# gvanhoy/gr-liquiddsp

Hardware: AMD Instinct MI355X
Metric: Msamples/s through flex_rx (QPSK r1/2 1024B) (higher is better)
Workload: dtype f32; 1 GPU; flex_rx single stream per GPU, 20000000 samples (10 Msym), PSK4 r=1/2 (CONV_V27), 1024-B payload, CRC-24, 256-sample gaps, CFO/phase/delay + AWGN Es/N0=20 dB; frames_decoded_ok=1154, streams_per_gpu=1, blocks_in_flight=12, stage_events=none (fxrx_set_timing level 0), steps=1415, passes=independent captures (reset between passes), segments=256, repairs=0

## Files before the change

### gr-liquiddsp_amd/csrc/fx_common.h

```cpp
#pragma once
#include <stdint.h>
#include <hip/hip_vector_types.h>

#define FX_K             2
#define FX_M             7
#define FX_BETA          0.3f
#define FX_NPFB          32
#define FX_MF_TAPS       28
#define FX_PROTO_LEN     897
#define FX_PN_LEN        64
#define FX_S_LEN         156
#define FX_NFFT          512
#define FX_HOP           256
#define FX_RANGE         24
#define FX_HDR_USER      14
#define FX_HDR_DEC       20
#define FX_HDR_CRC       24
#define FX_HDR_E0        27
#define FX_HDR_ENC       54
#define FX_HDR_MOD       216
#define FX_HDR_PILOTS    15
#define FX_HDR_SYM       231
#define FX_PILOT_SPACING 16
#define FX_PROTOCOL      102
// ... 220 lines not shown
    float2   sc[1024];
    uint32_t golenc[4096];
    uint16_t h128enc[256];
    uint8_t  h74enc[16], h84enc[16], sdcol[64], sd22col[16], sd39col[32];
    uint8_t  rsexp[512], rslog[256], rsgen[40];
    float2   pn[FX_PN_LEN], pilots[16];
};

struct FxChannel {
    uint32_t th0, dl;
    float    gain, sigma;
    uint64_t seed;
};

struct FxPayJob {
    const float2 *x, *xa_end;
    int64_t  start;
    uint32_t mix_th, mix_dl; float mf_scale;
    uint32_t pfb; int32_t mfc0;
    uint32_t pll_th; float pll_f;
    uint32_t ms, bps;
    uint32_t nsym;
    uint32_t sym_off;
    uint32_t pay_len, check, fec0, fec1;
    uint32_t k;
    uint32_t l0, l1;
    uint32_t byte_off;
    uint32_t dw_off;
    uint32_t out_off;
    uint32_t pad_;
    uint32_t eq;
    uint32_t chain_idx;
    uint32_t vb_off;
    uint16_t vb_nblk;
    uint16_t vb_clean;
};
static_assert(sizeof(FxPayJob) == 128, "FxPayJob: two 64-byte lines");

#ifndef FX_VB_WARM
#define FX_VB_WARM 96
#endif

struct FxPayResult {
    uint32_t stamp[8];
};

#define FX_GANG_MAX 4
struct FxPllMember {
    const FxPayJob *jobs; const uint32_t *pll_list; const FxBlockHdr *hdr; const float2 *sym_raw; float2 *framesyms; uint8_t *hard; FxOutRec *recs;
};
struct FxPllGang { uint32_t n; FxPllMember m[FX_GANG_MAX]; };
struct FxVbpreMember {
    FxPayJob *jobs; const uint32_t *job_idx; const FxBlockHdr *hdr; const uint8_t *hard; uint8_t *bufA, *bufB, *out; FxOutRec *recs; FxBlockHdr *hdr_host;
    uint32_t first_wave, n_waves;
};
struct FxVbpreGang { uint32_t n; FxVbpreMember m[FX_GANG_MAX]; };

struct FxPlanArgs {
    const FxStreamDesc *streams; uint32_t nstreams;
    uint32_t detect, eq;
    uint32_t vb_blk;
    const FxFrame *chain; const uint32_t *chain_count;
    uint32_t *stream_base;
    FxPayJob *pjobs; FxOutRec *recs;
    uint32_t *mf_job, *mf_c0, mf_cap;
    uint32_t *pll_list, *dec_list, list_cap;
    uint32_t *vb_items, vb_cap;
    FxBlockHdr *hdr, *hdr_pay, *hdr_host;
    uint32_t *ws;
};
```

### gr-liquiddsp_amd/csrc/fx_host.cpp

```cpp
#include <hip/hip_runtime.h>
#include <algorithm>
#include <chrono>
#include <cmath>
#include <cstdio>
#include <cstdlib>
#include <cstring>
#include <memory>
#include <string>
#include <vector>
#include "../../include/fxrx.h"
#include "fx_device.h"
#include "fx_codec.hpp"
#include "fx_launch.h"
#include "fx_traffic.h"

namespace {

thread_local std::string g_err;
void set_err(const std::string &s) { g_err = s; }

#define HIP_OK(expr)                                                                          \
    do {                                                                                      \
        hipError_t e_ = (expr);                                                               \
        if (e_ != hipSuccess) {                                                               \
// ... 657 lines not shown
    std::memcpy(sl.hp_desc.p + o_streams, sds.data(), NS * sizeof(FxStreamDesc));
    const uint32_t *d_list = sl.job_list();

    const double tp2 = g_prof_on ? prof_now() : 0.0;
    if (!sl.ingest.empty()) {
        std::vector<IngestJob> todo; todo.swap(sl.ingest);
        const size_t bytes = iq_sample_bytes(sl.ingest_fmt);
        for (const IngestJob &j : todo) {
            const void *src = j.dev_src;
            if (!src) { HIP_OK(hipMemcpyAsync(sl.d_raw[j.stream].p, j.host_src, j.n * bytes, hipMemcpyHostToDevice, st)); src = sl.d_raw[j.stream].p; }
            HIP_OK(fx_launch_ingest(st, sl.ingest_fmt, src, sl.d_in[j.stream].p, (size_t)j.n, sl.ingest_scale, (unsigned)c->n_cus));
        }
    }
    HIP_OK(fx_launch_upload(st, sl.hp_desc.p, sl.d_desc.p, desc_bytes, (unsigned)c->n_cus));
    const int tl = c->timing_level >= 0 ? c->timing_level : (c->depth > 1 ? 0 : 2);
    sl.timing_level = tl;
    if (c->debug_walk_twice > 0) HIP_OK(fx_launch_prescan(st, (unsigned)spec.size(), sl.ps_words, sl.jobs(), d_list + NJ, c->d_tables));
    for (int rep = 0; rep < c->debug_walk_twice; rep++) HIP_OK(launch_walk(c, sl, st, d_list, (unsigned)early.size()));
    if (tl >= 2) HIP_OK(hipEventRecord(sl.ev[kEvStart], st));
    if (c->debug_walk_twice <= 0) HIP_OK(fx_launch_prescan(st, (unsigned)spec.size(), sl.ps_words, sl.jobs(), d_list + NJ, c->d_tables));
    HIP_OK(launch_walk(c, sl, st, d_list, (unsigned)early.size()));
    const bool verify = !detect && c->skip_seek && !sl.force_noskip;
    hipStream_t cst = st;
    if (!late.empty()) {
        if (verify) {
            HIP_OK(fx_launch_copy_u32(st, &sl.hdr_walk()->n_runs, &sl.hdr_walk()->runs_done));
            HIP_OK(launch_seekverify(c, sl, st, c->verify_per_cu * (unsigned)c->n_cus, 0u));
        }
        if (!c->st_chain) {
            int lo = 0, hi = 0;
            HIP_OK(hipDeviceGetStreamPriorityRange(&lo, &hi));
            HIP_OK(hipStreamCreateWithPriority(&c->st_chain, hipStreamNonBlocking, hi));
        }
        HIP_OK(hipEventRecord(sl.ev[kEvHandover], st));
        cst = c->st_chain;
        HIP_OK(hipStreamWaitEvent(cst, sl.ev[kEvHandover], 0));
        if (c->prev_chain) HIP_OK(hipStreamWaitEvent(cst, c->prev_chain, 0));
        HIP_OK(launch_walk(c, sl, cst, d_list + early.size(), (unsigned)late.size()));
    }
    if (tl >= 2) HIP_OK(hipEventRecord(sl.ev[kEvWalk], cst));
    if (verify)
        HIP_OK(launch_seekverify(c, sl, cst, late.empty() ? c->verify_per_cu * (unsigned)c->n_cus : (unsigned)std::min<size_t>((size_t)c->verify_per_cu * (size_t)c->n_cus, std::max<size_t>(64, 16 * late.size())), 1u));
    if (tl >= 2) HIP_OK(hipEventRecord(sl.ev[kEvVerify], cst));
    if (late.empty() && c->prev_chain) HIP_OK(hipStreamWaitEvent(cst, c->prev_chain, 0));
    if (c->carry_reader[(b + 1) % 3]) HIP_OK(hipStreamWaitEvent(cst, c->carry_reader[(b + 1) % 3], 0));
    const double tp3 = g_prof_on ? prof_now() : 0.0;
    const int rb = enqueue_back(c, sl, kChainFast, cst, may_defer);
    if (g_prof_on) { const double tp4 = prof_now(); g_prof[1] += tp1 - tp0; g_prof[2] += tp2 - tp1; g_prof[3] += tp3 - tp2; g_prof[4] += tp4 - tp3; g_prof_n++; }
    return rb;
}

static FxVbpreMember vbpre_member(Slot &sl, uint32_t first_wave, uint32_t n_waves)
{
    return FxVbpreMember{ sl.d_pjobs.p, sl.dec_list(kDecBatch), sl.hdr_pay(), sl.d_hard.p, sl.d_bufA.p, sl.d_bufB.p, sl.h_out.p, sl.h_recs.p, sl.h_hdr.p, first_wave, n_waves };
}
static int launch_tails(fxrx_ctx_s *c, Slot *const *m, unsigned n)
{
    hipStream_t st = m[n - 1]->st;
    for (unsigned i = 0; i + 1 < n; i++) HIP_OK(hipStreamWaitEvent(st, m[i]->ev[kEvMf], 0));
    auto done = [&]() -> int {
        for (unsigned i = 0; i < n; i++) { HIP_OK(hipEventRecord(m[i]->ev[kEvDone], st)); m[i]->tail_launched = true; m[i]->tail_st = st; }
        if (n > 1) { c->gang_launches++; c->gang_members += n; }
        return 0;
    };
    {
        FxPllGang g; unsigned waves[FX_GANG_MAX]; g.n = n;
        for (unsigned i = 0; i < n; i++) { const Slot &sl = *m[i]; g.m[i] = FxPllMember{ sl.d_pjobs.p, sl.d_pll_list.p, sl.hdr_pay(), sl.d_symraw.p, sl.d_symraw.p, sl.d_hard.p, sl.h_recs.p }; waves[i] = sl.tail.pll_waves; }
        HIP_OK(fx_launch_paypll(&g, waves, c->pll_waves, st, c->d_tables));
    }
    for (unsigned i = 0; i < n; i++) if (m[i]->timing_level >= 1) HIP_OK(hipEventRecord(m[i]->ev[kEvPll], st));
    if (c->debug_stop_after == 6) return done();
    for (unsigned i = 0; i < n; i++) {
        Slot &sl = *m[i];
        if (c->cfg.soft_decision) {
            HIP_OK(fx_launch_softdemod(sl.tail.mf_grid, st, sl.d_pjobs.p, sl.d_mf_job.p, sl.d_mf_c0.p, sl.hdr_pay(), sl.d_symraw.p, sl.d_hard.p, sl.d_soft.p, c->d_tables));
            if (c->cfg.want_framesyms) HIP_OK(hipMemcpyAsync(sl.h_soft.p, sl.d_soft.p, 8 * sl.byte_cap, hipMemcpyDeviceToHost, st));
        }
        HIP_OK(launch_decoders(c, sl, st, 0u, sl.tail.plain, sl.tail.rs));
    }
    {
        FxVbpreGang g; g.n = n;
        for (unsigned i = 0; i < n; i++) g.m[i] = vbpre_member(*m[i], 0u, m[i]->vb_blk ? m[i]->tail.vb_pre : 0u);
        HIP_OK(fx_launch_vbpre(&g, st, c->d_tables, c->vb_clean ? 1 : 0, c->vb_early_tail && c->vb_clean ? 1 : 0));
    }
    for (unsigned i = 0; i < n; i++) {
        Slot &sl = *m[i];
        if (sl.vb_blk) HIP_OK(launch_trellis(c, sl, st, sl.tail.vb_items, sl.tail.vb_packed, sl.tail.with_fix, sl.tail.vb_fin, sl.tail.fb));
        if (sl.timing_level >= 2) HIP_OK(hipEventRecord(sl.ev[kEvDec], st));
        if (c->cfg.want_framesyms) HIP_OK(fx_launch_symcopy(2u * (unsigned)c->n_cus, st, sl.hdr_pay(), sl.d_symraw.p, sl.h_framesyms.p));
    }
    return done();
}

static int close_gang(fxrx_ctx_s *c)
{
    if (c->gang.empty()) return 0;
    if (c->gang.size() > FX_GANG_MAX) { set_err("open gang larger than FX_GANG_MAX (internal error)"); return FXRX_ERR_STATE; }
    Slot *m[FX_GANG_MAX]; unsigned n = 0;
    for (Slot *s : c->gang) m[n++] = s;
    c->gang.clear();
    return launch_tails(c, m, n);
}

static int enqueue_back(fxrx_ctx_s *c, Slot &sl, int chain_mode, hipStream_t chain_st, bool may_defer)
{
    const unsigned NS = c->cfg.n_streams; const bool detect = c->cfg.mode == FXRX_MODE_DETECTOR;
    const uint64_t b = sl.seq; const uint32_t chain_slots = sl.chain_cap; hipStream_t st = sl.st;
// ... 631 lines not shown
```

### gr-liquiddsp_amd/csrc/fx_kernels.hip

```cpp
#include <hip/hip_runtime.h>
#include <algorithm>
#include "fx_device.h"
#include "fx_launch.h"
#include "fx_vbclean.h"
#include "fx_rsgmd.h"

#define HALF         256

template <int WW> struct WalkLdsT {
    static constexpr int WAVES = WW;
    static constexpr bool SWEEP_PAIRS = WW == 4;
    float2 win[FX_NFFT];
    float2 X[FX_NFFT];
    float2 S[FX_NFFT];
    float2 scr[WW][576];
    float2 v[640];
    float2 P[256];
    float  m2[FX_NFFT];
    float2 hdr[FX_HDR_SYM];
    float2 cw[(WW + 1) * FX_HOP + 8];
    __device__ __forceinline__ float2 *scr2(int wave) { return wave < 2 ? v + 576 * wave : cw + 576 * (wave - 2); }
    float2 pb[16];
    float2 eqw[16];
    float  taps[FX_MF_TAPS];
// ... 1967 lines not shown
        __threadfence();
        __hip_atomic_store(&pw[PW_FLAG + wg], 2u, __ATOMIC_RELEASE, __HIP_MEMORY_SCOPE_AGENT);
    }
    __syncthreads();
    uint32_t before[PLAN_NV];
#pragma unroll
    for (int q = 0; q < PLAN_NV; q++) before[q] = base_s[q];
    for (uint32_t c0 = g0; c0 < g1; c0 += PLAN_THREADS) {
        const uint32_t g = c0 + tid;
        const bool live = g < g1;
        uint32_t v[PLAN_NV], tot[PLAN_NV]; PlanWords w;
        PlanFrame f = plan_frame(g, live, a, w, v);
        plan_scan<PLAN_THREADS>(v, tot, ws);
#pragma unroll
        for (int q = 0; q < PLAN_NV; q++) { v[q] += before[q]; before[q] += tot[q]; }
        if (f.batch && plan_demote(v[PV_VB], f.vnb, a.vb_cap)) { f.batch = false; f.vnb = 0; }
        if (live) {
            plan_emit(a.pjobs + g, a.recs + g, plan_rest(f.fp, a.streams + f.sidx), w, f, v, a.eq, (uint32_t)(f.fp - a.chain), 0u);
            for (uint32_t c = 0; c < f.nblk; c++) if (v[PV_MF] + c < a.mf_cap) { a.mf_job[v[PV_MF] + c] = g; a.mf_c0[v[PV_MF] + c] = c * 1024u; }
        }
        {
            const PlanKey key = plan_key(w.ms, w.fec0, w.fec1);
            (void)wave_agg_add(pw + PW_CLS_CNT, key.cls, 1u, f.valid);
            (void)wave_agg_add(pw + PW_DEC_CNT, key.dec(f.batch), 1u, f.valid);
            (void)wave_agg_add(pw + PW_VBC_CNT, key.vc, f.vnb, f.batch);
        }
        __syncthreads();
    }
}

extern "C" __global__ __launch_bounds__(PLAN_THREADS)
void fx_planlists_kernel(const FxPlanArgs a)
{
    __shared__ struct { FxBlockHdr h; uint32_t cls_base[FX_PLL_CLASSES + 1], vbc_base[8], last; } sh;
    uint32_t *const pw = a.ws;
    const PlanCounts<true> cnt{ pw + PW_CLS_CNT, pw + PW_DEC_CNT, pw + PW_VBC_CNT };
    const int tid = threadIdx.x;
    const uint32_t N = __hip_atomic_load(&a.stream_base[a.nstreams], __ATOMIC_RELAXED, __HIP_MEMORY_SCOPE_AGENT);
    if (tid == 0) plan_class_bases(cnt, sh.cls_base, sh.vbc_base);
    __syncthreads();
    uint32_t g0, g1; plan_range(N, g0, g1);
    for (uint32_t c0 = g0; c0 < g1; c0 += PLAN_THREADS) {
        const uint32_t g = c0 + tid;
        const bool live = g < g1;
        uint32_t ms = 0, fec0 = 0, fec1 = 0, vnb = 0; bool val = false;
        if (live) { const FxPayJob &j = a.pjobs[g]; val = j.pad_ != 0; ms = j.ms; fec0 = j.fec0; fec1 = j.fec1; vnb = j.vb_nblk; }
        const PlanKey key = plan_key(ms, fec0, fec1);
        const bool bt = val && vnb;
        const uint32_t pp = sh.cls_base[key.cls] + wave_agg_add(pw + PW_CLS_FILL, key.cls, 1u, val);
        if (val && pp < a.list_cap) a.pll_list[pp] = g;
        const uint32_t rs = key.dec(bt), dp = wave_agg_add(pw + PW_DEC_FILL, rs, 1u, val);
        if (val && dp < a.list_cap) a.dec_list[(size_t)rs * a.list_cap + dp] = g;
        const uint32_t at = sh.vbc_base[key.vc] + wave_agg_add(pw + PW_VBC_FILL, key.vc, vnb, bt);
        if (bt) {
            for (uint32_t b = 0; b < vnb; b++) if (at + b < a.vb_cap) { a.vb_items[at + b] = g; a.vb_items[a.vb_cap + at + b] = b; }
            a.pjobs[g].vb_off = at;
        }
    }
    if (blockIdx.x == 0) plan_pad_lists<PLAN_THREADS>(cnt, sh.cls_base, sh.vbc_base, a);
    __threadfence(); __syncthreads();
    if (tid == 0) sh.last = atomicAdd(&pw[PW_TICKET], 1u) == gridDim.x - 1 ? 1u : 0u;
    __syncthreads();
    if (!sh.last) return;
    __threadfence();
    if (tid == 0) {
        sh.h = *a.hdr;
        plan_fill_hdr(sh.h, N, (const volatile uint32_t *)(pw + PW_INC + 8 * (gridDim.x - 1)), cnt, sh.cls_base, sh.vbc_base, a);
    }
    __syncthreads();
    plan_mirror_hdr<PLAN_THREADS>(sh.h, a);
    for (int i = tid; i < PW_WORDS; i += PLAN_THREADS) pw[i] = 0u;
}

#define PLAN_TILE 2048
#define PLAN_BATCH 2
#define PLAN_LDS_STREAMS 256
enum { PO_CLS = 0, PO_DEC = FX_PLL_CLASSES, PO_VBC = FX_PLL_CLASSES + 4, PO_N = FX_PLL_CLASSES + 12 };
template <int NT> struct PlanOneShared {
    FxBlockHdr h;
    uint32_t ws[NT / 64][PLAN_NV];
    uint32_t cnt[PO_N], fill[PO_N];
    uint32_t cls_base[FX_PLL_CLASSES + 1], vbc_base[8];
    uint32_t sbase[PLAN_LDS_STREAMS + 1], cbase[PLAN_LDS_STREAMS];
};
template <int NT> __device__ __forceinline__ uint32_t plan_one_slot(uint32_t g, const FxPlanArgs &a, const PlanOneShared<NT> &sh, uint32_t &sidx)
{
    if (a.nstreams <= PLAN_LDS_STREAMS) { sidx = plan_stream_of(sh.sbase, a.nstreams, g); return sh.cbase[sidx] + (g - sh.sbase[sidx]); }
    sidx = plan_stream_of(a.stream_base, a.nstreams, g);
    return a.streams[sidx].chain_base + (g - a.stream_base[sidx]);
}

template <int NT> __global__ __launch_bounds__(NT)
void fx_planfused_kernel(const FxPlanArgs a)
{
    constexpr uint32_t TILE = PLAN_TILE;
    constexpr int KEEP = PLAN_TILE / NT, JB = PLAN_BATCH;
    static_assert(NT % 64 == 0 && KEEP * NT == PLAN_TILE && KEEP % JB == 0, "whole waves; the tile is KEEP frames a thread, in whole batches");
    __shared__ PlanOneShared<NT> sh;
    __shared__ uint4 keep[PLAN_TILE];
    const PlanCounts<false> cnt{ sh.cnt + PO_CLS, sh.cnt + PO_DEC, sh.cnt + PO_VBC };
    const uint32_t tid = threadIdx.x, nstreams = a.nstreams;
#ifdef FX_STAMPS
    unsigned long long tk_ = __builtin_readcyclecounter(); uint32_t st1_ = 0, st2_ = 0, st6_ = 0, st7_ = 0;
#define PLAN_TICK(acc) do { const unsigned long long t_ = __builtin_readcyclecounter(); acc += (uint32_t)(t_ - tk_); tk_ = t_; } while (0)
#else
#define PLAN_TICK(acc) do { } while (0)
#endif
    {
        const uint32_t *src = reinterpret_cast<const uint32_t *>(a.hdr); uint32_t *dst = reinterpret_cast<uint32_t *>(&sh.h);
        for (int i = (int)tid; i < (int)(sizeof(FxBlockHdr) / 4); i += NT) dst[i] = src[i];
        if (tid < PO_N) { sh.cnt[tid] = 0u; sh.fill[tid] = 0u; }
        if (tid <= FX_PLL_CLASSES) sh.cls_base[tid] = 0u;
        if (tid < 8) sh.vbc_base[tid] = 0u;
    }
    uint32_t N;
    if (nstreams <= PLAN_LDS_STREAMS) {
        uint32_t v[PLAN_NV] = { tid < nstreams ? a.chain_count[tid] : 0u, 0, 0, 0, 0, 0, 0 }, tot[PLAN_NV];
        if (nstreams > 1) plan_scan<NT>(v, tot, sh.ws); else { tot[0] = v[0]; v[0] = 0u; }
        if (tid < nstreams) { sh.sbase[tid] = v[0]; a.stream_base[tid] = v[0]; sh.cbase[tid] = a.streams[tid].chain_base; }
        if (tid == 0) { sh.sbase[nstreams] = tot[0]; a.stream_base[nstreams] = tot[0]; }
        __syncthreads();
        N = sh.sbase[nstreams];
    } else N = plan_stream_bases<NT>(a.chain_count, nstreams, a.stream_base, sh.ws);

    uint32_t run[PLAN_NV] = { 0, 0, 0, 0, 0, 0, 0 };
    for (int pass = N > TILE ? 0 : 1; pass < 2; pass++) {
#pragma unroll
        for (int q = 0; q < PLAN_NV; q++) run[q] = 0u;
        for (uint32_t t0 = 0; t0 < N; t0 += TILE) {
            const uint32_t nt = min(TILE, N - t0), t1 = t0 + nt, per = (nt + NT - 1) / NT, f0 = t0 + tid * per;
            uint32_t st[PLAN_NV];
            PlanWords w[KEEP]; uint32_t slot[KEEP], sidx[KEEP];
#pragma unroll
            for (int i = 0; i < KEEP; i++) {
                const bool live = (uint32_t)i < per && f0 + i < t1;
                slot[i] = plan_one_slot(live ? f0 + i : t0, a, sh, sidx[i]);
                w[i] = plan_words(a.chain + slot[i]);
            }
#pragma unroll
            for (int q = 0; q < PLAN_NV; q++) st[q] = 0u;
#pragma unroll
            for (int i = 0; i < KEEP; i++) {
                uint32_t v[PLAN_NV];
                (void)plan_sizes(w[i], (uint32_t)i < per && f0 + i < t1, a.detect, a.vb_blk, v);
#pragma unroll
                for (int q = 0; q < PLAN_NV; q++) st[q] += v[q];
            }
            {
                uint32_t tot[PLAN_NV];
                plan_scan<NT>(st, tot, sh.ws);
#pragma unroll
                for (int q = 0; q < PLAN_NV; q++) { st[q] += run[q]; run[q] += tot[q]; }
            }
            if (pass == 0 || N <= TILE) {
                uint32_t vb = st[PV_VB];
#pragma unroll
                for (int i = 0; i < KEEP; i++) {
                    uint32_t v[PLAN_NV];
                    const PlanFrame f = plan_sizes(w[i], (uint32_t)i < per && f0 + i < t1, a.detect, a.vb_blk, v);
                    const bool batch = f.batch && !plan_demote(vb, f.vnb, a.vb_cap);
                    vb += f.vnb;
                    if (f.valid) {
                        const PlanKey key = plan_key(w[i].ms, w[i].fec0, w[i].fec1);
                        atomicAdd(&sh.cnt[PO_CLS + key.cls], 1u);
                        atomicAdd(&sh.cnt[PO_DEC + key.dec(batch)], 1u);
                        if (batch) atomicAdd(&sh.cnt[PO_VBC + key.vc], f.vnb);
                    }
                }
            }
            if (pass == 0) continue;
            if (t0 == 0) {
                __syncthreads();
                if (tid == 0) plan_class_bases(cnt, sh.cls_base, sh.vbc_base);
                __syncthreads();
            }
            PLAN_TICK(st1_);
#pragma unroll
            for (int b0 = 0; b0 < KEEP; b0 += JB) {
                if ((uint32_t)b0 >= per) break;
                PlanRest r[JB];
#pragma unroll
                for (int i = 0; i < JB; i++) r[i] = plan_rest(a.chain + slot[b0 + i], a.streams + sidx[b0 + i]);
#pragma unroll
                for (int i = 0; i < JB; i++) {
                    const uint32_t g = f0 + b0 + i;
                    if ((uint32_t)(b0 + i) >= per || g >= t1) break;
                    const PlanWords &wi = w[b0 + i];
                    uint32_t v[PLAN_NV];
                    PlanFrame f = plan_sizes(wi, true, a.detect, a.vb_blk, v);
                    f.fp = a.chain + slot[b0 + i]; f.sidx = sidx[b0 + i];
                    if (f.batch && plan_demote(st[PV_VB], f.vnb, a.vb_cap)) { f.batch = false; f.vnb = 0; }
                    uint32_t at = 0;
                    if (f.valid) {
                        const PlanKey key = plan_key(wi.ms, wi.fec0, wi.fec1);
                        const uint32_t pp = sh.cls_base[key.cls] + atomicAdd(&sh.fill[PO_CLS + key.cls], 1u);
                        if (pp < a.list_cap) a.pll_list[pp] = g;
                        const uint32_t rs = key.dec(f.batch), dp = atomicAdd(&sh.fill[PO_DEC + rs], 1u);
                        if (dp < a.list_cap) a.dec_list[(size_t)rs * a.list_cap + dp] = g;
                        if (f.batch) at = sh.vbc_base[key.vc] + atomicAdd(&sh.fill[PO_VBC + key.vc], f.vnb);
                    }
                    keep[g - t0] = make_uint4(at, f.vnb, st[PV_MF], f.nblk);
                    plan_emit(a.pjobs + g, a.recs + g, r[i], wi, f, st, a.eq, slot[b0 + i], at);
#pragma unroll
                    for (int q = 0; q < PLAN_NV; q++) st[q] += v[q];
                }
            }
            __syncthreads();
            PLAN_TICK(st2_);
            for (uint32_t k = tid >> 4; k < nt; k += NT / 16) {
                const uint4 kp = keep[k];
                const uint32_t g = t0 + k, sub = tid & 15u;
                for (uint32_t b = sub; b < kp.y; b += 16u) if (kp.x + b < a.vb_cap) { a.vb_items[kp.x + b] = g; a.vb_items[a.vb_cap + kp.x + b] = b; }
                for (uint32_t c = sub; c < kp.w; c += 16u) if (kp.z + c < a.mf_cap) { a.mf_job[kp.z + c] = g; a.mf_c0[kp.z + c] = c * 1024u; }
            }
            __syncthreads();
        }
    }
    plan_pad_lists<NT>(cnt, sh.cls_base, sh.vbc_base, a);
    PLAN_TICK(st6_);
    __threadfence(); __syncthreads();
    PLAN_TICK(st7_);
    if (tid == 0) {
#ifdef FX_STAMPS
        sh.h.stamp[1] = st1_; sh.h.stamp[2] = st2_; sh.h.stamp[6] = st6_; sh.h.stamp[7] = st7_;
#endif
        plan_fill_hdr(sh.h, N, run, cnt, sh.cls_base, sh.vbc_base, a);
    }
    __syncthreads();
    plan_mirror_hdr<NT>(sh.h, a);
}

extern "C" hipError_t fx_launch_plan(hipStream_t st, unsigned grid, int fused, unsigned threads, const FxPlanArgs &a)
{
    const unsigned g = grid < 1u ? 1u : (grid > PLAN_MAXG ? PLAN_MAXG : grid);
    if (fused && g == 1u) {
        if (threads == 512u) hipLaunchKernelGGL((fx_planfused_kernel<512>), dim3(1), dim3(512), 0, st, a);
        else if (threads == 256u) hipLaunchKernelGGL((fx_planfused_kernel<256>), dim3(1), dim3(256), 0, st, a);
        else return hipErrorInvalidValue;
    } else {
        hipLaunchKernelGGL(fx_plan_kernel, dim3(g), dim3(PLAN_THREADS), 0, st, a);
        hipLaunchKernelGGL(fx_planlists_kernel, dim3(g), dim3(PLAN_THREADS), 0, st, a);
    }
    return hipGetLastError();
}
extern "C" unsigned fx_plan_ws_words(void) { return PW_WORDS; }

#define PMF_THREADS 256
#define PMF_SYMS    1024
#define PMF_SPAN    (2 * PMF_SYMS + FX_MF_TAPS)

__global__ __launch_bounds__(PMF_THREADS)
void fx_paymf_kernel(const FxPayJob *jobs, const uint32_t *blk_job, const uint32_t *blk_c0, const FxBlockHdr *hdr, const FxFrame *chain, float2 *sym_raw,
                     const FxTables *T)
{
    constexpr int LEAD = FX_EQ_TAPS - 1;
    __shared__ float2 v[PMF_SPAN + LEAD + 4];
    __shared__ float2 u[2 * PMF_SYMS + FX_EQ_TAPS];
    __shared__ float2 eqw[16];
    __shared__ float taps[FX_MF_TAPS];
    const uint32_t nitems = hdr->n_mfblk;
    const int tid = threadIdx.x;
    const float2 *sc = T->sc;
    for (uint32_t bi = blockIdx.x; bi < nitems; bi += gridDim.x) {
        const FxPayJob job = jobs[blk_job[bi]];
        const uint32_t c0 = blk_c0[bi];
        const uint32_t ns = min((uint32_t)PMF_SYMS, job.nsym - c0);
// ... 1575 lines not shown
    row[8] = q2.x; row[9] = q2.y; row[10] = q2.z; row[11] = q2.w; row[12] = q3.x; row[13] = q3.y; row[14] = q3.z; row[15] = q3.w;
    lbase = o << 3;
}
__device__ __forceinline__ void vb2_forward(int p, uint32_t blk, const VbHalf &A, const VbHalf &B, uint32_t *lds)
{
    uint32_t Q[64], N[64];
#pragma unroll
    for (int i = 0; i < 64; i++) Q[i] = 0u;
    unsigned pa, pb; conv_punct(p, pa, pb);
    const unsigned up = (unsigned)p;
    const uint32_t warm = vb_warm(p);
    VbStream sa = vb_stream_at(A.first ? A.t_reg : A.t_reg - warm, up), sb = vb_stream_at(B.first ? B.t_reg : B.t_reg - warm, up);
    const auto lo = [&](int i) { return (Q[i] & 0xFFFFu) >> 1; };
    const auto hi = [&](int i) { return Q[i] >> 17; };
    uint32_t *rowa = lds + (threadIdx.x & 63) * VB_ROW, *rowb = lds + (64 + (threadIdx.x & 63)) * VB_ROW;
    uint32_t la = 0, lb = 0;
    const uint32_t nsteps = warm + blk;
    for (uint32_t u = 0; u < nsteps; u += 2) {
        if (u == warm) {
            if (A.first) {
#pragma unroll
                for (int i = 0; i < 64; i++) Q[i] = (Q[i] & 0xFFFF0000u) | (i ? 1024u : 0u);
            } else if (A.on) vb_save_vec(lo, A.vec);
            if (B.first) {
#pragma unroll
                for (int i = 0; i < 64; i++) Q[i] = (Q[i] & 0x0000FFFFu) | (i ? 1024u << 16 : 0u);
            } else if (B.on) vb_save_vec(hi, B.vec);
        }
        if ((u & 127u) == 0u) { vb_stage(A.enc, sa.nb, A.on, rowa, la); vb_stage(B.enc, sb.nb, B.on, rowb, lb); }
        if ((u & 15u) == 0u) {
            const uint32_t ia = (sa.nb - la) >> 5, ib = (sb.nb - lb) >> 5;
            sa.w0 = __builtin_bswap32(rowa[ia]); sa.w1 = __builtin_bswap32(rowa[ia + 1]); sa.wbase = la + (ia << 5);
            sb.w0 = __builtin_bswap32(rowb[ib]); sb.w1 = __builtin_bswap32(rowb[ib + 1]); sb.wbase = lb + (ib << 5);
        }
        const bool in_reg = u >= warm;
        const bool run_a = in_reg || !A.first, run_b = in_reg || !B.first;
        unsigned long long a0, b0, a1, b1;
        vb2_step(Q, N, pa, pb, up, sa, sb, run_a, run_b, a0, b0);
        vb2_step(N, Q, pa, pb, up, sa, sb, run_a, run_b, a1, b1);
        const uint32_t ur = u - warm;
        if (in_reg && ur < (uint32_t)FX_VB_TWARM) {
            if (A.on && A.t_reg + ur < A.t1) { A.dwl[(size_t)ur * 64u] = a0; A.dwl[(size_t)(ur + 1u) * 64u] = a1; }
            if (B.on && B.t_reg + ur < B.t1) { B.dwl[(size_t)ur * 64u] = b0; B.dwl[(size_t)(ur + 1u) * 64u] = b1; }
        } else {
            if (A.on && in_reg && A.t_reg + ur < A.t1) { __builtin_nontemporal_store(a0, A.dwl + (size_t)ur * 64u); __builtin_nontemporal_store(a1, A.dwl + (size_t)(ur + 1u) * 64u); }
            if (B.on && in_reg && B.t_reg + ur < B.t1) { __builtin_nontemporal_store(b0, B.dwl + (size_t)ur * 64u); __builtin_nontemporal_store(b1, B.dwl + (size_t)(ur + 1u) * 64u); }
        }
    }
    if (A.on) vb_save_vec(lo, A.vec + 64);
    if (B.on) vb_save_vec(hi, B.vec + 64);
}

struct VbItem { uint32_t g, b, t_reg, t1, Tn, nblk; bool on; };
__device__ __forceinline__ VbItem vb_item(const FxPayJob *jobs, const uint32_t *vb_items, uint32_t item_cap, uint32_t slot, uint32_t blk)
{
    VbItem it;
    const uint32_t item = vb_items[slot];
    it.on = item != 0xFFFFFFFFu;
    it.g = it.on ? item : 0u; it.b = it.on ? vb_items[item_cap + slot] : 0u;
    const FxPayJob &job = jobs[it.g];
    it.on = it.on && job.vb_clean == 0u;
    it.Tn = 8u * job.k + 6u; it.nblk = job.vb_nblk;
    it.t_reg = it.b * blk; it.t1 = min(it.Tn, it.t_reg + blk);
    return it;
}
struct VbWaveItem { VbItem it; uint32_t slot; unsigned long long *dwl; uint8_t *vec; };
__device__ __forceinline__ VbWaveItem vb_wave_item(const FxPayJob *jobs, const uint32_t *vb_items, uint32_t item_cap, uint32_t slot, uint32_t blk,
                                                   unsigned long long *dwv, uint8_t *vec_arena)
{
    VbWaveItem w;
    w.slot = slot; w.it = vb_item(jobs, vb_items, item_cap, slot, blk);
    w.dwl = vb_slab(dwv, slot, blk); w.vec = vec_arena ? vec_arena + (size_t)slot * 128u : nullptr;
    return w;
}
__device__ __forceinline__ int vb_wave_period(unsigned long long live, unsigned fec0)
{
    return conv_p((unsigned)__shfl((int)fec0, __ffsll((long long)live) - 1, 64));
}

extern "C" __global__ __launch_bounds__(64, 3)
void fx_vbfwd_kernel(const FxPayJob *jobs, const uint32_t *vb_items, uint32_t item_cap, const FxBlockHdr *hdr, uint32_t first_item, const uint8_t *bufB,
                     unsigned long long *dwv, uint8_t *vec_arena, uint32_t *vb_st)
{
    const uint32_t nitems = hdr->n_vb_items, blk = hdr->vb_blk;
    const uint32_t it0 = first_item + blockIdx.x * 128u;
    if (it0 >= nitems) return;
    const uint32_t slot_a = it0 + threadIdx.x, slot_b = slot_a + 64u;
    const VbItem ia = vb_item(jobs, vb_items, item_cap, slot_a, blk);
    VbItem ib = ia; ib.on = false;
    if (slot_b < nitems) ib = vb_item(jobs, vb_items, item_cap, slot_b, blk);
    const unsigned long long live_a = __ballot(ia.on), live_b = __ballot(ib.on);
    if (!live_a && !live_b) return;
    const FxPayJob &ja = jobs[ia.g], &jb = jobs[ib.g];
    const int p = live_a ? vb_wave_period(live_a, ja.fec0) : vb_wave_period(live_b, jb.fec0);
    VbHalf A, B;
    A.enc = bufB + ja.byte_off; A.on = ia.on; A.first = !ia.on || ia.b == 0; A.t_reg = A.first && !ia.on ? 0u : ia.t_reg; A.t1 = ia.t1;
    A.dwl = vb_slab(dwv, slot_a, blk); A.vec = vec_arena + (size_t)slot_a * 128u;
    B.enc = bufB + jb.byte_off; B.on = ib.on; B.first = !ib.on || ib.b == 0; B.t_reg = B.first && !ib.on ? 0u : ib.t_reg; B.t1 = ib.t1;
    B.dwl = vb_slab(dwv, ib.on ? slot_b : slot_a, blk); B.vec = vec_arena + (size_t)(ib.on ? slot_b : slot_a) * 128u;
    __shared__ uint32_t rows[128 * VB_ROW];
    vb2_forward(p, blk, A, B, rows);
    if (ia.on) vb_st[slot_a] = vb_st_fresh(vb_make_guess(A.dwl, ia.t1 - ia.t_reg), false);
    if (ib.on) vb_st[slot_b] = vb_st_fresh(vb_make_guess(B.dwl, ib.t1 - ib.t_reg), false);
}

extern "C" __global__ __launch_bounds__(64)
void fx_vbfwd1_kernel(const FxPayJob *jobs, const uint32_t *vb_items, uint32_t item_cap, const FxBlockHdr *hdr, uint32_t first_item, const uint8_t *bufB,
                      unsigned long long *dwv, uint8_t *vec_arena, uint32_t *vb_st)
{
    const uint32_t nitems = hdr->n_vb_items, blk = hdr->vb_blk;
    const uint32_t it0 = first_item + blockIdx.x * 64u;
    if (it0 >= nitems) return;
    const VbWaveItem w = vb_wave_item(jobs, vb_items, item_cap, it0 + threadIdx.x, blk, dwv, vec_arena);
    const VbItem &it = w.it;
    const unsigned long long live = __ballot(it.on);
    if (!live) return;
    const FxPayJob &job = jobs[it.g];
    const int p = vb_wave_period(live, job.fec0);
    const bool first = !it.on || it.b == 0;
    vb_forward(bufB + job.byte_off, p, it.t_reg, it.t1, first ? 1 : 0, nullptr, w.dwl, first ? nullptr : w.vec, w.vec + 64,
               vb_warm(p) + blk, vb_warm(p), it.on);
    if (it.on) vb_st[w.slot] = vb_st_fresh(vb_make_guess(w.dwl, it.t1 - it.t_reg), false);
}

__device__ __forceinline__ bool vb_same64(const uint8_t *a, const uint8_t *b)
{
    const uint4 *pa = reinterpret_cast<const uint4 *>(a), *pb = reinterpret_cast<const uint4 *>(b);
    bool same = true;
#pragma unroll
    for (int i = 0; i < 4; i++) { const uint4 x = pa[i], y = pb[i]; same = same && x.x == y.x && x.y == y.y && x.z == y.z && x.w == y.w; }
    return same;
}

extern "C" __global__ __launch_bounds__(64)
void fx_vbfix_kernel(const FxPayJob *jobs, const uint32_t *vb_items, uint32_t item_cap, const FxBlockHdr *hdr, uint32_t first_item, const uint8_t *bufB,
                     unsigned long long *dwv, uint8_t *vec_arena, uint32_t *vb_st, uint32_t dbg)
{
    const uint32_t nitems = hdr->n_vb_items, blk = hdr->vb_blk;
    const uint32_t it0 = first_item + blockIdx.x * 64u;
    if (it0 >= nitems) return;
    const VbWaveItem w = vb_wave_item(jobs, vb_items, item_cap, it0 + threadIdx.x, blk, dwv, vec_arena);
    const VbItem &it = w.it;
    uint8_t *vec = w.vec;
    const bool bad = it.on && it.b > 0 && !vb_same64(vec, vec - 64) && !((dbg & 2u) && (w.slot & 1u));
    const unsigned long long fails = __ballot(bad);
    if (!fails) return;
    const FxPayJob &job = jobs[it.g];
    const int p = vb_wave_period(fails, job.fec0);
    vb_forward(bufB + job.byte_off, p, it.t_reg, it.t1, 2, bad ? vec - 64 : vec, w.dwl, vec, vec + 64, blk, 0u, bad);
    if (bad) vb_st[w.slot] = vb_st_fresh(vb_make_guess(w.dwl, it.t1 - it.t_reg), true);
}

__device__ __forceinline__ void vb_trace16(const unsigned long long *dwl, uint32_t u0, uint32_t lim, unsigned &st, uint32_t &bits16)
{
    unsigned long long q[16];
#pragma unroll
    for (int i = 0; i < 16; i++) q[i] = (u0 + (uint32_t)i < lim) ? dwl[(size_t)(u0 + (uint32_t)i) * 64u] : 0ull;
#pragma unroll
    for (int i = 15; i >= 0; i--) {
        if (u0 + (uint32_t)i < lim) {
            bits16 |= (st & 1u) << i;
            st = (st >> 1) | ((unsigned)((q[i] >> st) & 1ull) << 5);
        }
    }
}
__device__ __forceinline__ unsigned vb_trace_chunk(const unsigned long long *dwl, uint32_t c, uint32_t len, unsigned st, uint32_t &b0, uint32_t &b1)
{
    unsigned long long bits = 0;
#pragma unroll 1
    for (int grp = 3; grp >= 0; grp--) {
        uint32_t b16 = 0;
        vb_trace16(dwl, 64u * c + 16u * (uint32_t)grp, len, st, b16);
        bits |= (unsigned long long)b16 << (16 * grp);
    }
    b0 = (uint32_t)bits; b1 = (uint32_t)(bits >> 32);
    return st;
}

extern "C" __global__ __launch_bounds__(64)
void fx_vbtrace_kernel(const FxPayJob *jobs, const uint32_t *vb_items, uint32_t item_cap, const FxBlockHdr *hdr, uint32_t first_item, uint8_t *bufA,
                       unsigned long long *dwv, uint32_t *vb_st, uint32_t dbg)
{
    const uint32_t nitems = hdr->n_vb_items, blk = hdr->vb_blk;
    const uint32_t it0 = first_item + blockIdx.x * 64u;
    if (it0 >= nitems) return;
    const VbWaveItem w = vb_wave_item(jobs, vb_items, item_cap, it0 + threadIdx.x, blk, dwv, nullptr);
    const VbItem &it = w.it;
    const uint32_t slot = w.slot;
    if (!__ballot(it.on)) return;
    const FxPayJob &job = jobs[it.g];
    const uint32_t len = it.on ? it.t1 - it.t_reg : 0u;
    const uint32_t old = it.on ? vb_st[slot] : 0u;
    const unsigned long long *dwl = w.dwl;
    const bool has_next = it.on && it.b + 1u < it.nblk;
    const unsigned S = (has_next && !(dbg & 1u)) ? vb_st_guess(vb_st[slot + 1u]) : 0u;
    uint8_t *A = bufA + job.byte_off + it.t_reg / 8u;
    unsigned st = S;
    for (int c = (int)(blk / 64u) - 1; c >= 0; c--) {
        if (!__any(64u * (uint32_t)c < len)) continue;
        uint32_t b0, b1;
        st = vb_trace_chunk(dwl, (uint32_t)c, len, st, b0, b1);
        if (64u * (uint32_t)c < len) vb_emit(A, (uint32_t)c, b0, b1);
    }
    if (it.on) vb_st[slot] = vb_st_traced(old, S, st);
}

struct VbSlabTracer {
    static constexpr uint32_t max_chunks = 64u;
    const unsigned long long *dwl; uint32_t len;
    template <int NCH>
    __device__ __forceinline__ void operator()(const uint32_t (&cidx)[NCH], const bool (&act)[NCH], unsigned (&st)[NCH], uint32_t (&bits)[NCH][2]) const
    {
#pragma unroll
        for (int j = 0; j < NCH; j++) if (act[j]) st[j] = vb_trace_chunk(dwl, cidx[j], len, st[j], bits[j][0], bits[j][1]);
    }
};
__device__ __forceinline__ unsigned vb_retrace_block(const unsigned long long *dwl, uint32_t len, unsigned end_state, uint8_t *dec, uint8_t *scratch, int lane)
{
    const VbSlabTracer trace = { dwl, len };
    const unsigned arrived = vb_traceback<1>(trace, (len + 63) / 64, end_state, dec, scratch, lane);
    __threadfence_block(); __builtin_amdgcn_wave_barrier();
    return arrived;
}

template <bool IN_LDS>
__device__ __forceinline__ void vbpre_front(const FxPayJob &job, const uint8_t *hs, uint8_t *X, uint8_t *A, uint8_t *B, const FxTables *T, int lane)
{
    uint8_t *W = IN_LDS ? X : A;
    pack_bytes_wave(hs, job.bps, job.l1, W, lane);
    if (!IN_LDS) __threadfence_block();
    __builtin_amdgcn_wave_barrier();
    deinterleave_wave(W, job.l1, lane);
    if (!IN_LDS || job.fec1 != FX_FEC_NONE) {
        if (IN_LDS) {
            for (uint32_t j = lane; j < job.l1; j += DEC_THREADS) A[j] = X[j];
            __threadfence_block(); __builtin_amdgcn_wave_barrier();
        }
        block_fec_decode<false>(job.fec1, job.l0, A, B, T, lane);
        __threadfence_block(); __builtin_amdgcn_wave_barrier();
        if (IN_LDS) {
            for (uint32_t j = lane; j < job.l0; j += DEC_THREADS) X[j] = B[j];
            __builtin_amdgcn_wave_barrier();
        } else W = B;
    }
    deinterleave_wave(W, job.l0, lane);
    if (lane < (IN_LDS ? 16 : 8)) W[job.l0 + lane] = 0;
}
__device__ __forceinline__ uint64_t vb_lds_word(const uint8_t *X, uint32_t w)
{
    const uint2 v = reinterpret_cast<const uint2 *>(X)[w];
    return ((uint64_t)__builtin_bswap32(v.x) << 32) | __builtin_bswap32(v.y);
}
__device__ __forceinline__ bool vb_clean_check(FxPayJob *jobs, uint32_t jf, uint32_t k, const uint8_t *X, uint8_t *A, int lane)
{
    const uint32_t Tn = 8u * k + 6u, nw = (Tn + 31u) / 32u;
    bool ok = true;
    for (uint32_t w = lane; w < nw; w += DEC_THREADS) {
        uint32_t u;
        ok = ok && vbc_check_word(w >= 2u ? vb_lds_word(X, w - 2u) : 0ull, w >= 1u ? vb_lds_word(X, w - 1u) : 0ull, vb_lds_word(X, w), w, Tn, u) == 0u;
    }
    const bool clean = !__any(!ok);
    if (clean) {
        for (uint32_t w = lane; 4u * w < k; w += DEC_THREADS) {
            uint32_t u;
            (void)vbc_check_word(w >= 2u ? vb_lds_word(X, w - 2u) : 0ull, w >= 1u ? vb_lds_word(X, w - 1u) : 0ull, vb_lds_word(X, w), w, Tn, u);
            reinterpret_cast<uint32_t *>(A)[w] = __builtin_bswap32(u);
        }
    }
    if (lane == 0) jobs[jf].vb_clean = clean ? 1u : 0u;
    return clean;
}
extern "C" __global__ __launch_bounds__(DEC_THREADS)
void fx_vbpre_kernel(const FxVbpreGang g, const FxTables *T, uint32_t clean_on, uint32_t early_tail)
{
    __shared__ __attribute__((aligned(16))) uint8_t X[DEC_LDS];
    const FxVbpreMember m = g.m[blockIdx.y];
    if (blockIdx.x >= m.n_waves) return;
    const uint32_t njobs = m.hdr->n_dec_batch;
    const uint32_t ji = m.first_wave + blockIdx.x;
    if (ji >= njobs) return;
    FxPayJob *jobs = m.jobs; const uint8_t *hard = m.hard; uint8_t *bufA = m.bufA, *bufB = m.bufB, *out = m.out;
    FxOutRec *recs = m.recs; FxBlockHdr *hdr_host = m.hdr_host;
    const int lane = threadIdx.x & 63;
    const uint32_t jf = m.job_idx[ji];
    FxPayJob job = jobs[jf];
    job.l0 = __builtin_amdgcn_readfirstlane(job.l0); job.l1 = __builtin_amdgcn_readfirstlane(job.l1);
    job.fec1 = __builtin_amdgcn_readfirstlane(job.fec1); job.bps = __builtin_amdgcn_readfirstlane(job.bps);
    uint8_t *A = bufA + job.byte_off, *B = bufB + job.byte_off;
    const uint8_t *hs = hard + job.sym_off;
    if (vbpre_lds_fits(job.l1, job.l0)) {
        vbpre_front<true>(job, hs, X, A, B, T, lane);
        __builtin_amdgcn_wave_barrier();
        const uint32_t n16 = (job.l0 + 8u + 15u) / 16u;
        for (uint32_t j = lane; j < n16; j += DEC_THREADS) reinterpret_cast<uint4 *>(B)[j] = reinterpret_cast<const uint4 *>(X)[j];
        job.k = __builtin_amdgcn_readfirstlane(job.k);
        const bool clean = clean_on && conv_p(job.fec0) == 1 && vb_clean_check(jobs, jf, job.k, X, A, lane);
        if (!early_tail) return;
        if (!clean) { if (lane == 0) hdr_host->vb_dirty = 1u; return; }
        job.pay_len = __builtin_amdgcn_readfirstlane(job.pay_len); job.check = __builtin_amdgcn_readfirstlane(job.check);
        __threadfence_block(); __builtin_amdgcn_wave_barrier();
        dec_tail(job, jf, A, lane, out, recs, FX_REC_VB_CLEAN);
        return;
    }
    vbpre_front<false>(job, hs, nullptr, A, B, T, lane);
    if (early_tail && lane == 0) hdr_host->vb_dirty = 1u;
}

extern "C" __global__ __launch_bounds__(64)
void fx_vbfinish_kernel(const FxPayJob *jobs, const uint32_t *job_idx, FxBlockHdr *hdr, uint32_t first_wave, uint8_t *bufA, uint8_t *bufB,
                        unsigned long long *dwv, const uint8_t *vec_arena, const uint32_t *vb_st, uint32_t *fb_list, uint32_t list_cap, uint8_t *out, FxOutRec *recs,
                        FxBlockHdr *hdr_host, uint32_t early_tail)
{
    const uint32_t njobs = hdr->n_dec_batch, blk = hdr->vb_blk;
    const uint32_t ji = first_wave + blockIdx.x;
    if (ji >= njobs) return;
    const int lane = threadIdx.x & 63;
    const uint32_t jf = job_idx[ji];
    FxPayJob job = jobs[jf];
    job.k = __builtin_amdgcn_readfirstlane(job.k); job.pay_len = __builtin_amdgcn_readfirstlane(job.pay_len);
    job.check = __builtin_amdgcn_readfirstlane(job.check); job.vb_nblk = (uint16_t)__builtin_amdgcn_readfirstlane(job.vb_nblk);
    job.vb_off = __builtin_amdgcn_readfirstlane(job.vb_off); job.vb_clean = (uint16_t)__builtin_amdgcn_readfirstlane(job.vb_clean);
    uint8_t *A = bufA + job.byte_off, *B = bufB + job.byte_off;
    if (job.vb_clean) { if (!early_tail) dec_tail(job, jf, A, lane, out, recs, FX_REC_VB_CLEAN); return; }
    const uint32_t at = job.vb_off, nblk = job.vb_nblk;
    bool bad = false, mism = false; uint32_t rep = 0;
    for (uint32_t base = 0; base < nblk; base += 64) {
        const uint32_t b = base + (uint32_t)lane;
        const uint32_t v = b < nblk ? vb_st[at + b] : 0u, vn = b + 1u < nblk ? vb_st[at + b + 1u] : 0u;
        if (b > 0 && b < nblk) { const uint8_t *vec = vec_arena + (size_t)(at + b) * 128u; const bool same = vb_same64(vec, vec - 64); bad = bad || !same; }
        rep += (uint32_t)__popcll(__ballot(vb_st_repeated(v)));
        mism = mism || (b + 1u < nblk && vb_st_end(v) != vb_st_arrived(vn));
    }
    if (__any(bad)) {
        if (lane == 0) { const uint32_t s = atomicAdd(&hdr->n_vb_fallback, 1u); if (s < list_cap) fb_list[s] = jf; hdr_host->vb_ticket = 1u; }
        return;
    }
    if (__any(mism)) {
        unsigned need = vb_st_arrived(vb_st[at + nblk - 1u]);
        for (int b = (int)nblk - 2; b >= 0; b--) {
            const uint32_t v = vb_st[at + (uint32_t)b];
            if (vb_st_end(v) != need) need = vb_retrace_block(vb_slab(dwv, at + (uint32_t)b, blk), blk, need, A + (size_t)b * (blk / 8u), B, lane);
            else need = vb_st_arrived(v);
        }
    }
    __threadfence_block(); __builtin_amdgcn_wave_barrier();
    dec_tail(job, jf, A, lane, out, recs, rep << 8);
}

extern "C" hipError_t fx_launch_vbpre(const FxVbpreGang *gang, hipStream_t st, const FxTables *T, int clean_on, int early_tail)
{
    if (gang->n > FX_GANG_MAX) return hipErrorInvalidValue;
    FxVbpreGang g; g.n = 0;
    unsigned gw = 0;
    for (uint32_t i = 0; i < gang->n; i++) if (gang->m[i].n_waves) { g.m[g.n++] = gang->m[i]; gw = gang->m[i].n_waves > gw ? gang->m[i].n_waves : gw; }
    if (g.n == 0) return hipSuccess;
    for (uint32_t i = g.n; i < FX_GANG_MAX; i++) g.m[i] = g.m[0];
    hipLaunchKernelGGL(fx_vbpre_kernel, dim3(gw, g.n), dim3(DEC_THREADS), 0, st, g, T, clean_on ? 1u : 0u, early_tail ? 1u : 0u);
// ... 405 lines not shown
```

Measured before the change: 40680 Msamples/s.

## Write Viterbi block item lists in vbpre, skipping entries for clean frames

```diff
diff --git a/gr-liquiddsp_amd/csrc/fx_common.h b/gr-liquiddsp_amd/csrc/fx_common.h
--- a/gr-liquiddsp_amd/csrc/fx_common.h
+++ b/gr-liquiddsp_amd/csrc/fx_common.h
@@ -296,6 +296,7 @@
 struct FxPllGang { uint32_t n; FxPllMember m[FX_GANG_MAX]; };
 struct FxVbpreMember {
     FxPayJob *jobs; const uint32_t *job_idx; const FxBlockHdr *hdr; const uint8_t *hard; uint8_t *bufA, *bufB, *out; FxOutRec *recs; FxBlockHdr *hdr_host;
+    uint32_t *vb_items; uint32_t vb_cap;
     uint32_t first_wave, n_waves;
 };
 struct FxVbpreGang { uint32_t n; FxVbpreMember m[FX_GANG_MAX]; };
diff --git a/gr-liquiddsp_amd/csrc/fx_host.cpp b/gr-liquiddsp_amd/csrc/fx_host.cpp
--- a/gr-liquiddsp_amd/csrc/fx_host.cpp
+++ b/gr-liquiddsp_amd/csrc/fx_host.cpp
@@ -733,7 +733,7 @@
 
 static FxVbpreMember vbpre_member(Slot &sl, uint32_t first_wave, uint32_t n_waves)
 {
-    return FxVbpreMember{ sl.d_pjobs.p, sl.dec_list(kDecBatch), sl.hdr_pay(), sl.d_hard.p, sl.d_bufA.p, sl.d_bufB.p, sl.h_out.p, sl.h_recs.p, sl.h_hdr.p, first_wave, n_waves };
+    return FxVbpreMember{ sl.d_pjobs.p, sl.dec_list(kDecBatch), sl.hdr_pay(), sl.d_hard.p, sl.d_bufA.p, sl.d_bufB.p, sl.h_out.p, sl.h_recs.p, sl.h_hdr.p, sl.d_vb_items.p, sl.vb_cap, first_wave, n_waves };
 }
 static int launch_tails(fxrx_ctx_s *c, Slot *const *m, unsigned n)
 {
diff --git a/gr-liquiddsp_amd/csrc/fx_kernels.hip b/gr-liquiddsp_amd/csrc/fx_kernels.hip
--- a/gr-liquiddsp_amd/csrc/fx_kernels.hip
+++ b/gr-liquiddsp_amd/csrc/fx_kernels.hip
@@ -2043,10 +2043,7 @@
         const uint32_t rs = key.dec(bt), dp = wave_agg_add(pw + PW_DEC_FILL, rs, 1u, val);
         if (val && dp < a.list_cap) a.dec_list[(size_t)rs * a.list_cap + dp] = g;
         const uint32_t at = sh.vbc_base[key.vc] + wave_agg_add(pw + PW_VBC_FILL, key.vc, vnb, bt);
-        if (bt) {
-            for (uint32_t b = 0; b < vnb; b++) if (at + b < a.vb_cap) { a.vb_items[at + b] = g; a.vb_items[a.vb_cap + at + b] = b; }
-            a.pjobs[g].vb_off = at;
-        }
+        if (bt) a.pjobs[g].vb_off = at;
     }
     if (blockIdx.x == 0) plan_pad_lists<PLAN_THREADS>(cnt, sh.cls_base, sh.vbc_base, a);
     __threadfence(); __syncthreads();
@@ -2088,7 +2085,7 @@
     constexpr int KEEP = PLAN_TILE / NT, JB = PLAN_BATCH;
     static_assert(NT % 64 == 0 && KEEP * NT == PLAN_TILE && KEEP % JB == 0, "whole waves; the tile is KEEP frames a thread, in whole batches");
     __shared__ PlanOneShared<NT> sh;
-    __shared__ uint4 keep[PLAN_TILE];
+    __shared__ uint2 keep[PLAN_TILE];
     const PlanCounts<false> cnt{ sh.cnt + PO_CLS, sh.cnt + PO_DEC, sh.cnt + PO_VBC };
     const uint32_t tid = threadIdx.x, nstreams = a.nstreams;
 #ifdef FX_STAMPS
@@ -2190,7 +2187,7 @@
                         if (dp < a.list_cap) a.dec_list[(size_t)rs * a.list_cap + dp] = g;
                         if (f.batch) at = sh.vbc_base[key.vc] + atomicAdd(&sh.fill[PO_VBC + key.vc], f.vnb);
                     }
-                    keep[g - t0] = make_uint4(at, f.vnb, st[PV_MF], f.nblk);
+                    keep[g - t0] = make_uint2(st[PV_MF], f.nblk);
                     plan_emit(a.pjobs + g, a.recs + g, r[i], wi, f, st, a.eq, slot[b0 + i], at);
 #pragma unroll
                     for (int q = 0; q < PLAN_NV; q++) st[q] += v[q];
@@ -2199,10 +2196,9 @@
             __syncthreads();
             PLAN_TICK(st2_);
             for (uint32_t k = tid >> 4; k < nt; k += NT / 16) {
-                const uint4 kp = keep[k];
+                const uint2 kp = keep[k];
                 const uint32_t g = t0 + k, sub = tid & 15u;
-                for (uint32_t b = sub; b < kp.y; b += 16u) if (kp.x + b < a.vb_cap) { a.vb_items[kp.x + b] = g; a.vb_items[a.vb_cap + kp.x + b] = b; }
-                for (uint32_t c = sub; c < kp.w; c += 16u) if (kp.z + c < a.mf_cap) { a.mf_job[kp.z + c] = g; a.mf_c0[kp.z + c] = c * 1024u; }
+                for (uint32_t c = sub; c < kp.y; c += 16u) if (kp.x + c < a.mf_cap) { a.mf_job[kp.x + c] = g; a.mf_c0[kp.x + c] = c * 1024u; }
             }
             __syncthreads();
         }
@@ -3884,24 +3880,26 @@
 }
 
 struct VbItem { uint32_t g, b, t_reg, t1, Tn, nblk; bool on; };
-__device__ __forceinline__ VbItem vb_item(const FxPayJob *jobs, const uint32_t *vb_items, uint32_t item_cap, uint32_t slot, uint32_t blk)
+__device__ __forceinline__ VbItem vb_item(const FxPayJob *jobs, const uint32_t *vb_items, uint32_t item_cap, uint32_t slot, uint32_t blk, uint32_t nframes)
 {
     VbItem it;
     const uint32_t item = vb_items[slot];
-    it.on = item != 0xFFFFFFFFu;
-    it.g = it.on ? item : 0u; it.b = it.on ? vb_items[item_cap + slot] : 0u;
+    it.on = item < nframes;
+    it.g = it.on ? item : 0u;
     const FxPayJob &job = jobs[it.g];
-    it.on = it.on && job.vb_clean == 0u;
+    const uint32_t b = slot - job.vb_off;
+    it.on = it.on && job.vb_clean == 0u && b < job.vb_nblk && vb_items[item_cap + slot] == b;
+    it.b = it.on ? b : 0u;
     it.Tn = 8u * job.k + 6u; it.nblk = job.vb_nblk;
     it.t_reg = it.b * blk; it.t1 = min(it.Tn, it.t_reg + blk);
     return it;
 }
 struct VbWaveItem { VbItem it; uint32_t slot; unsigned long long *dwl; uint8_t *vec; };
-__device__ __forceinline__ VbWaveItem vb_wave_item(const FxPayJob *jobs, const uint32_t *vb_items, uint32_t item_cap, uint32_t slot, uint32_t blk,
+__device__ __forceinline__ VbWaveItem vb_wave_item(const FxPayJob *jobs, const uint32_t *vb_items, uint32_t item_cap, uint32_t slot, uint32_t blk, uint32_t nframes,
                                                    unsigned long long *dwv, uint8_t *vec_arena)
 {
     VbWaveItem w;
-    w.slot = slot; w.it = vb_item(jobs, vb_items, item_cap, slot, blk);
+    w.slot = slot; w.it = vb_item(jobs, vb_items, item_cap, slot, blk, nframes);
     w.dwl = vb_slab(dwv, slot, blk); w.vec = vec_arena ? vec_arena + (size_t)slot * 128u : nullptr;
     return w;
 }
@@ -3914,13 +3912,13 @@
 void fx_vbfwd_kernel(const FxPayJob *jobs, const uint32_t *vb_items, uint32_t item_cap, const FxBlockHdr *hdr, uint32_t first_item, const uint8_t *bufB,
                      unsigned long long *dwv, uint8_t *vec_arena, uint32_t *vb_st)
 {
-    const uint32_t nitems = hdr->n_vb_items, blk = hdr->vb_blk;
+    const uint32_t nitems = hdr->n_vb_items, blk = hdr->vb_blk, nframes = hdr->n_frames;
     const uint32_t it0 = first_item + blockIdx.x * 128u;
     if (it0 >= nitems) return;
     const uint32_t slot_a = it0 + threadIdx.x, slot_b = slot_a + 64u;
-    const VbItem ia = vb_item(jobs, vb_items, item_cap, slot_a, blk);
+    const VbItem ia = vb_item(jobs, vb_items, item_cap, slot_a, blk, nframes);
     VbItem ib = ia; ib.on = false;
-    if (slot_b < nitems) ib = vb_item(jobs, vb_items, item_cap, slot_b, blk);
+    if (slot_b < nitems) ib = vb_item(jobs, vb_items, item_cap, slot_b, blk, nframes);
     const unsigned long long live_a = __ballot(ia.on), live_b = __ballot(ib.on);
     if (!live_a && !live_b) return;
     const FxPayJob &ja = jobs[ia.g], &jb = jobs[ib.g];
@@ -3940,10 +3938,10 @@
 void fx_vbfwd1_kernel(const FxPayJob *jobs, const uint32_t *vb_items, uint32_t item_cap, const FxBlockHdr *hdr, uint32_t first_item, const uint8_t *bufB,
                       unsigned long long *dwv, uint8_t *vec_arena, uint32_t *vb_st)
 {
-    const uint32_t nitems = hdr->n_vb_items, blk = hdr->vb_blk;
+    const uint32_t nitems = hdr->n_vb_items, blk = hdr->vb_blk, nframes = hdr->n_frames;
     const uint32_t it0 = first_item + blockIdx.x * 64u;
     if (it0 >= nitems) return;
-    const VbWaveItem w = vb_wave_item(jobs, vb_items, item_cap, it0 + threadIdx.x, blk, dwv, vec_arena);
+    const VbWaveItem w = vb_wave_item(jobs, vb_items, item_cap, it0 + threadIdx.x, blk, nframes, dwv, vec_arena);
     const VbItem &it = w.it;
     const unsigned long long live = __ballot(it.on);
     if (!live) return;
@@ -3968,10 +3966,10 @@
 void fx_vbfix_kernel(const FxPayJob *jobs, const uint32_t *vb_items, uint32_t item_cap, const FxBlockHdr *hdr, uint32_t first_item, const uint8_t *bufB,
                      unsigned long long *dwv, uint8_t *vec_arena, uint32_t *vb_st, uint32_t dbg)
 {
-    const uint32_t nitems = hdr->n_vb_items, blk = hdr->vb_blk;
+    const uint32_t nitems = hdr->n_vb_items, blk = hdr->vb_blk, nframes = hdr->n_frames;
     const uint32_t it0 = first_item + blockIdx.x * 64u;
     if (it0 >= nitems) return;
-    const VbWaveItem w = vb_wave_item(jobs, vb_items, item_cap, it0 + threadIdx.x, blk, dwv, vec_arena);
+    const VbWaveItem w = vb_wave_item(jobs, vb_items, item_cap, it0 + threadIdx.x, blk, nframes, dwv, vec_arena);
     const VbItem &it = w.it;
     uint8_t *vec = w.vec;
     const bool bad = it.on && it.b > 0 && !vb_same64(vec, vec - 64) && !((dbg & 2u) && (w.slot & 1u));
@@ -4013,10 +4011,10 @@
 void fx_vbtrace_kernel(const FxPayJob *jobs, const uint32_t *vb_items, uint32_t item_cap, const FxBlockHdr *hdr, uint32_t first_item, uint8_t *bufA,
                        unsigned long long *dwv, uint32_t *vb_st, uint32_t dbg)
 {
-    const uint32_t nitems = hdr->n_vb_items, blk = hdr->vb_blk;
+    const uint32_t nitems = hdr->n_vb_items, blk = hdr->vb_blk, nframes = hdr->n_frames;
     const uint32_t it0 = first_item + blockIdx.x * 64u;
     if (it0 >= nitems) return;
-    const VbWaveItem w = vb_wave_item(jobs, vb_items, item_cap, it0 + threadIdx.x, blk, dwv, nullptr);
+    const VbWaveItem w = vb_wave_item(jobs, vb_items, item_cap, it0 + threadIdx.x, blk, nframes, dwv, nullptr);
     const VbItem &it = w.it;
     const uint32_t slot = w.slot;
     if (!__ballot(it.on)) return;
@@ -4083,7 +4081,7 @@
     const uint2 v = reinterpret_cast<const uint2 *>(X)[w];
     return ((uint64_t)__builtin_bswap32(v.x) << 32) | __builtin_bswap32(v.y);
 }
-__device__ __forceinline__ bool vb_clean_check(FxPayJob *jobs, uint32_t jf, uint32_t k, const uint8_t *X, uint8_t *A, int lane)
+__device__ __forceinline__ bool vb_clean_check(uint32_t k, const uint8_t *X, uint8_t *A, int lane)
 {
     const uint32_t Tn = 8u * k + 6u, nw = (Tn + 31u) / 32u;
     bool ok = true;
@@ -4099,8 +4097,16 @@
             reinterpret_cast<uint32_t *>(A)[w] = __builtin_bswap32(u);
         }
     }
-    if (lane == 0) jobs[jf].vb_clean = clean ? 1u : 0u;
     return clean;
+}
+__device__ __forceinline__ void vb_write_run(uint32_t *vb_items, uint32_t item_cap, uint32_t g, uint32_t at, uint32_t nblk, bool clean, int lane)
+{
+    for (uint32_t b = lane; b < nblk; b += DEC_THREADS) {
+        const uint32_t slot = at + b;
+        if (slot >= item_cap) break;
+        vb_items[slot] = clean ? 0xFFFFFFFFu : g;
+        if (!clean) vb_items[item_cap + slot] = b;
+    }
 }
 extern "C" __global__ __launch_bounds__(DEC_THREADS)
 void fx_vbpre_kernel(const FxVbpreGang g, const FxTables *T, uint32_t clean_on, uint32_t early_tail)
@@ -4126,7 +4132,10 @@
         const uint32_t n16 = (job.l0 + 8u + 15u) / 16u;
         for (uint32_t j = lane; j < n16; j += DEC_THREADS) reinterpret_cast<uint4 *>(B)[j] = reinterpret_cast<const uint4 *>(X)[j];
         job.k = __builtin_amdgcn_readfirstlane(job.k);
-        const bool clean = clean_on && conv_p(job.fec0) == 1 && vb_clean_check(jobs, jf, job.k, X, A, lane);
+        const bool checked = clean_on && conv_p(job.fec0) == 1;
+        const bool clean = checked && vb_clean_check(job.k, X, A, lane);
+        vb_write_run(m.vb_items, m.vb_cap, jf, job.vb_off, job.vb_nblk, clean, lane);
+        if (checked && lane == 0) jobs[jf].vb_clean = clean ? 1u : 0u;
         if (!early_tail) return;
         if (!clean) { if (lane == 0) hdr_host->vb_dirty = 1u; return; }
         job.pay_len = __builtin_amdgcn_readfirstlane(job.pay_len); job.check = __builtin_amdgcn_readfirstlane(job.check);
@@ -4135,6 +4144,7 @@
         return;
     }
     vbpre_front<false>(job, hs, nullptr, A, B, T, lane);
+    vb_write_run(m.vb_items, m.vb_cap, jf, job.vb_off, job.vb_nblk, false, lane);
     if (early_tail && lane == 0) hdr_host->vb_dirty = 1u;
 }
 
```

After: 45340 Msamples/s, median of 6. 11.5% higher.
